# genome/breakdancer

Measured on AMD Instinct MI355X. Metric: read-pairs/s, records resident in HBM -> scored SV table (SURVEY 8d timing i); end to end from BAM: config.timings.bam_to_table (vs_baseline is taken there), higher is better.
Workload: dtype int32

## Files before the change

### breakdancer_amd/_lib.py

```python
import ctypes as C
import os

import numpy as np

_HERE = os.path.dirname(os.path.abspath(__file__))
LIB_PATH = os.path.join(_HERE, "libbdx.so")

OPT_FIELDS = ["min_len", "cut_sd", "max_sd", "min_map_qual", "min_read_pair", "seq_coverage_lim", "buffer_size",
              "transchr_rearrange", "fisher", "illumina_long_insert", "cn_lib", "print_af", "score_threshold",
              "chr_restricted"]


class bdx_opts(C.Structure):
    _fields_ = [(k, C.c_int32) for k in OPT_FIELDS]


class bdx_lib(C.Structure):
    _fields_ = [("mean_insertsize", C.c_float), ("std_insertsize", C.c_float), ("uppercutoff", C.c_float),
                ("lowercutoff", C.c_float), ("readlens", C.c_float), ("min_mapping_quality", C.c_int32),
                ("bam_index", C.c_int32)]


class bdx_batch(C.Structure):
    _fields_ = [(k, C.c_void_p) for k in ("tid", "pos", "mtid", "mpos", "isize", "flag", "qlen", "mapq", "lib", "bam",
# ... 11 lines not shown
                ("n_groups", C.c_uint32), ("n_svs", C.c_uint32), ("n_svs_printed", C.c_uint32)]


REGION_DTYPE = np.dtype([("tid", "<i4"), ("start", "<i4"), ("end", "<i4"), ("normal_read_pairs", "<i4"),
                         ("fwd_read_count", "<i4"), ("rev_read_count", "<i4"), ("n_reads", "<i4"), ("stored", "<i4"),
                         ("max_qlen", "<i4")])
SV_DTYPE = np.dtype([("chr", "<i4", 2), ("pos", "<i4", 2), ("fwd", "<i4", 2), ("rev", "<i4", 2), ("flag", "<i4"),
                     ("size", "<i4"), ("score", "<i4"), ("num_reads", "<i4"), ("printed", "<i4"), ("region", "<i4", 2),
                     ("lib_begin", "<i4"), ("lib_count", "<i4"), ("cn_begin", "<i4"), ("cn_count", "<i4"),
                     ("allele_frequency", "<f4"), ("logp", "<f8")])

EXPORTS = ["bdx_opts_default", "bdx_create", "bdx_destroy", "bdx_strerror", "bdx_last_error", "bdx_reserve", "bdx_push",
           "bdx_set_device_reads", "bdx_run", "bdx_get_summary", "bdx_get_counters", "bdx_get_regions", "bdx_get_svs",
           "bdx_get_sv_lists", "bdx_get_read_class", "bdx_get_timings", "bdx_classify", "bdx_poisson_log_upper_tail",
           "bdx_device", "bdx_stream", "bdx_set_collect_support", "bdx_get_sv_support",
           "bdx_set_host_walk", "bdx_set_debug", "bdx_use_name_check", "bdx_run_many", "bdx_get_walk_split", "bdx_trim_results", "bdx_set_stage_timing", "bdx_get_cross_window_svs",
           "bdx_set_enqueue_ahead", "bdx_was_replayed", "bdx_acquire_batch", "bdx_submit_batch", "bdx_reset_reads", "bdx_set_pass1_statistics",
           "bdx_warm_up", "bdx_set_process_option", "bdx_dist_unique_id", "bdx_dist_create", "bdx_dist_create_threads", "bdx_dist_destroy", "bdx_dist_last_error", "bdx_dist_rank",
           "bdx_dist_world", "bdx_dist_chromosome", "bdx_dist_run", "bdx_dist_result", "bdx_dist_set_collect_support", "bdx_dist_get_phase_ms", "bdx_dist_phase_name", "bdx_dist_prepare", "bdx_dist_reset_reads", "bdx_dist_get_exchange", "bdx_dist_get_collectives", "bdx_dist_set_debug", "bdx_dist_owner", "bdx_dist_plan",
           "bdx_bamdec_create", "bdx_bamdec_destroy", "bdx_bamdec_last_error", "bdx_bamdec_acquire", "bdx_bamdec_submit", "bdx_bamdec_progress",
           "bdx_bamdec_finish", "bdx_bamdec_rearm", "bdx_bamdec_fetch", "bdx_bamdec_stats", "bdx_bamdec_host_ms", "bdx_merge_decoded", "bdx_append_decoded", "bdx_inflate_blocks", "bdx_insert_size_stats",
           "bdx_count_junction_pairs", "bdx_bamdec_set_exclude", "bdx_bamdec_excluded", "bdx_exclude_mask", "bdx_count_site_pairs", "bdx_site_breakpoint_bounds", "bdx_count_interval_reads",
           "bdx_set_mark_duplicates", "bdx_get_duplicates", "bdx_dist_set_mark_duplicates", "bdx_dist_get_duplicates", "bdx_mark_duplicates"]

DUP_T = 64

SITE_DTYPE = np.dtype([("tid1", "<i4"), ("pos1", "<i4"), ("tid2", "<i4"), ("pos2", "<i4"), ("flag_mask", "<u4")])
SITE_BOUNDS_DTYPE = np.dtype([("n", "<u4"), ("lo1", "<i4"), ("hi1", "<i4"), ("lo2", "<i4"), ("hi2", "<i4")])
INTERVAL_DTYPE = np.dtype([("tid", "<i4"), ("beg", "<i4"), ("end", "<i4")])
DEPTH_CHUNK = 2048
SITE_FLAGS = (1 << 1) | (1 << 2) | (1 << 3) | (1 << 4) | (1 << 5) | (1 << 8)
# ... 32 lines not shown
    L.bdx_get_read_class.argtypes = [vp, vp, C.c_size_t]
    L.bdx_get_timings.argtypes = [vp, vp, C.c_int]
    L.bdx_set_host_walk.argtypes = [vp, C.c_int]
    L.bdx_set_debug.argtypes = [vp, C.c_char_p, C.c_int]
    L.bdx_use_name_check.argtypes = [vp, C.c_int]
    L.bdx_run_many.argtypes = [C.POINTER(vp), C.c_size_t, C.c_int]
    L.bdx_set_stage_timing.argtypes = [vp, C.c_int]
    L.bdx_set_enqueue_ahead.argtypes = [vp, C.c_int]
    L.bdx_was_replayed.argtypes = [vp]
    L.bdx_acquire_batch.argtypes = [vp, C.c_size_t, C.POINTER(bdx_batch_buf)]
    L.bdx_submit_batch.argtypes = [vp, C.c_size_t]
    L.bdx_reset_reads.argtypes = [vp]
    L.bdx_set_pass1_statistics.argtypes = [vp, vp, C.c_uint32]
    L.bdx_get_walk_split.argtypes = [vp, vp, vp, vp]
    L.bdx_get_cross_window_svs.argtypes = [vp, vp]
    L.bdx_classify.argtypes = [C.POINTER(bdx_opts), C.POINTER(bdx_lib), C.c_int, C.POINTER(bdx_batch), vp, C.c_int]
    L.bdx_poisson_log_upper_tail.argtypes = [vp, vp, vp, C.c_size_t, C.c_int]
    L.bdx_device.argtypes = [vp]
    L.bdx_stream.argtypes = [vp]
    L.bdx_stream.restype = vp
    L.bdx_set_collect_support.argtypes = [vp, C.c_int]
    L.bdx_get_sv_support.argtypes = [vp, vp, vp, vp, C.c_size_t, vp]
    L.bdx_count_junction_pairs.argtypes = [vp, vp, vp, vp, C.c_size_t, C.c_int, vp]
    L.bdx_count_site_pairs.argtypes = [vp, vp, C.c_size_t, C.c_int32, C.c_int, vp]
    L.bdx_site_breakpoint_bounds.argtypes = [vp, vp, C.c_size_t, C.c_int32, vp]
    L.bdx_count_interval_reads.argtypes = [vp, vp, C.c_size_t, C.c_int, vp]
    L.bdx_set_mark_duplicates.argtypes = [vp, C.c_int]
    L.bdx_get_duplicates.argtypes = [vp, vp, vp]
    L.bdx_dist_set_mark_duplicates.argtypes = [vp, C.c_int]
    L.bdx_dist_get_duplicates.argtypes = [vp, vp, vp]
# ... 4 lines not shown
```

### breakdancer_amd/api.py

```python
import ctypes as C
from dataclasses import dataclass

import numpy as np

from . import _lib as L

FLAG_NAMES = ["NA", "ARP_FF", "ARP_LARGE_INSERT", "ARP_SMALL_INSERT", "ARP_RF", "ARP_RR", "NORMAL_FR", "NORMAL_RF",
              "ARP_CTX", "MATE_UNMAPPED", "UNMAPPED"]


class BdxError(RuntimeError):
    pass


@dataclass
class Options:
    min_len: int = 7
    cut_sd: int = 3
    max_sd: int = 1000000000
    min_map_qual: int = 35
    min_read_pair: int = 2
    seq_coverage_lim: int = 1000
    buffer_size: int = 100
    transchr_rearrange: bool = False
# ... 301 lines not shown
        return self

    def walk_split(self):
        v = [C.c_uint32(0), C.c_uint32(0), C.c_uint32(0)]
        self._chk(self.lib.bdx_get_walk_split(self.h, C.byref(v[0]), C.byref(v[1]), C.byref(v[2])), "bdx_get_walk_split")
        return tuple(x.value for x in v)

    def was_replayed(self):
        return bool(self.lib.bdx_was_replayed(self.h))

    def cross_window_svs(self):
        v = C.c_uint32(0)
        self._chk(self.lib.bdx_get_cross_window_svs(self.h, C.byref(v)), "bdx_get_cross_window_svs")
        return v.value

    def timings(self):
        ms = np.zeros(12, np.float32)
        self.lib.bdx_get_timings(self.h, ms.ctypes.data_as(C.c_void_p), 12)
        return dict(zip(("classify", "compact", "regions", "join", "readback", "walk", "score", "total", "final_wait", "merge",
                         "combine_scores"), ms.tolist()))


def mark_duplicates(tid, pos, mtid, mpos, flag, lib, name_key, device=0):
    lb = L.load()
    cols = [np.ascontiguousarray(a, dtype=dt) for a, dt in ((tid, np.int32), (pos, np.int32), (mtid, np.int32), (mpos, np.int32),
                                                            (flag, np.uint16), (lib, np.uint8), (name_key, np.uint64))]
    n = len(cols[0])
    if any(len(c) != n for c in cols):
        raise ValueError("the columns differ in length")
    out = np.zeros(n, np.uint8)
# ... 18 lines not shown
```

### breakdancer_amd/csrc/bdx_api.hip

```cpp
#include <hip/hip_runtime.h>

#include <algorithm>
#include <atomic>
#include <functional>
#include <memory>
#include <chrono>
#include <cmath>
#include <cstdio>
#include <cstddef>
#include <cstring>
#include <string>
#include <thread>
#include <unordered_map>
#include <utility>
#include <vector>

#include "../../include/bdx.h"
#include "bdx_buf.h"
#include "bdx_dev.h"
#include "bdx_k3.h"
#include "bdx_shard.h"
#include "bdx_scan.h"
#include "bdx_walk.h"
#include "bdx_bam_dev.h"
// ... 38 lines not shown
    size_t n = 0, cap = 0;
    bool adopted = false;
    DevBuf b_tid, b_pos, b_mtid, b_mpos, b_isize, b_flag, b_qlen, b_mapq, b_lib, b_bam, b_key, b_check;
    bool groups_in_hbm = false;
    bool use_check = false;

    DevBuf b_libs, b_cls, b_tile_tot, b_tile_pre, b_tile_mono, b_blk_cnt, b_cnt, b_p1, b_fold, b_stash, b_chunk_tot, b_counts;
    DevBuf b_lib_mean, b_kdens;
    PinBuf h_p1, h_cnt, h_counts, h_terms;
    PinBuf h_hs_rec, h_hs_aux, h_hs_lists, h_printed;
    StageBufs sb;
    PinBuf h_flags;
    PinBuf h_count;
    uint32_t seq = 0;
    int dbg_no_stash = 0, dbg_max_chunks = 0, dbg_ins_plain = 0, dbg_gather_walk = 0, dbg_regions_copy = 0, dbg_asm_plain = 0, dbg_depth_plain = 0;
    uint32_t lb_seq = 0;
    float k1_ms_last = 0;
    bool k1_timed = false;
    bool stage_timing = false;
    bool poll = true;
    bool materialized = true;
    bool rows_packed = false;
    uint32_t n_sv_total = 0, n_groups_total = 0, n_terms_total = 0, n_cn_total = 0;
    Event ev_groups, ev_regions;
    int big_walk_mode = -1;
    int64_t last_big_groups = -1;
    FinalizeParams fp_deferred{};
    bool finalize2_deferred = false;
    bool bucketed_join = false;
    bool host_walk_only = false;
// ... 178 lines not shown

StageDims stage_dims(const bdx_ctx* c, uint32_t na) {
    StageDims d;
    d.na = na; d.nkeys = c->nkeys; d.nlibs = c->nlibs; d.use_check = c->use_check;
    d.k2_clears_join = c->force_direct_join || (!c->bucketed_join && na <= kDirectJoinMax);
    d.groups_in_hbm = c->groups_in_hbm; d.table_in_hbm = c->table_in_hbm; d.k6_cap = c->k6_cap;
    d.big_walk = c->big_walk_mode >= 0 ? c->big_walk_mode : (c->last_big_groups >= 0 ? (c->last_big_groups > 2000 ? 1 : 0) : -1);
    d.join_n = d.join_own = na; d.join_slots = d.k2_clears_join ? direct_join_slots(na) : 0;
    return d;
}

int pass1_prepare(bdx_ctx* c, uint32_t tiles_cap);
int presize_stages(bdx_ctx* c, const StageDims& dm);
int presize_stages_here(bdx_ctx* c, const StageDims& dm);
int pass1_classify(bdx_ctx* c, uint32_t upto, bool timed);

constexpr uint32_t kStreamTilesMin = 4096;

int enqueue_batch(bdx_ctx* c, const bdx_batch& b, bool lazy_keys) {
    if (c->n + b.n > c->cap) {
        BDX_TRY(alloc_reads(c, std::max(c->n + b.n, c->cap * 2)));
    }
    const size_t o = c->n, n = b.n;
    if (c->mark_dup && c->dup_done && o)
        return fail(c, BDX_ESTATE, "duplicates of this load are marked already: reads cannot be appended behind a run (bdx_reset_reads starts the next load)");
    hipStream_t s = c->copy_stream;
    if (o == 0) {
        c->key_segs.clear();
        const uint64_t tiles = (c->cap + kTile - 1) / kTile;
        if (tiles <= 0xFFFFFFFFull) {
// ... 391 lines not shown
    c->k1_done = 0;
    HIPCHK(c, c->b_cls.ensure(std::max<size_t>((size_t)tiles_cap * kTile, 16)));
    c->use_stash = !c->dbg_no_stash && nkeys <= kStashKeys;
    if (c->use_stash) HIPCHK(c, c->b_stash.ensure(std::max<size_t>((size_t)tiles_cap * kStashCap * sizeof(StashRec), 64)));
    HIPCHK(c, c->b_tile_tot.ensure((size_t)ncols * tstride * 4));
    HIPCHK(c, c->b_tile_pre.ensure((size_t)ncols * tstride * 4));
    HIPCHK(c, c->b_tile_mono.ensure((size_t)nbams * tstride * sizeof(MonoRec)));
    HIPCHK(c, c->b_blk_cnt.ensure((size_t)kCntCopies * ncnt * 4));
    HIPCHK(c, c->b_cnt.ensure((size_t)ncnt * 4));
    HIPCHK(c, c->b_p1.ensure(sizeof(Pass1)));
    HIPCHK(c, c->h_p1.ensure(sizeof(Pass1)));
    HIPCHK(c, c->h_cnt.ensure((size_t)ncnt * 4));
    HIPCHK(c, c->h_counts.ensure(sizeof(StageCounts)));
    HIPCHK(c, c->b_counts.ensure(sizeof(StageCounts)));
    HIPCHK(c, c->h_count.ensure((size_t)kMaxChunks * 8));
    const size_t w_tot = (size_t)ncols * tstride, w_mono = (size_t)nbams * tstride * sizeof(MonoRec) / 4;
    if (w_tot > 0xFFFFFFFFull || w_mono > 0xFFFFFFFFull) {
        HIPCHK(c, hipMemsetAsync(c->b_tile_tot.p, 0, w_tot * 4, s));
        HIPCHK(c, hipMemsetAsync(c->b_tile_mono.p, 0xFF, w_mono * 4, s));
    }
    InitList il{};
    int k = 0;
    auto add = [&](void* p, size_t words, uint32_t value) { il.ptr[k] = (uint32_t*)p; il.words[k] = (uint32_t)words; il.value[k] = value; ++k; };
    if (w_tot <= 0xFFFFFFFFull && w_mono <= 0xFFFFFFFFull) { add(c->b_tile_tot.p, w_tot, 0u); add(c->b_tile_mono.p, w_mono, 0xFFFFFFFFu); }
    add(c->b_blk_cnt.p, (size_t)kCntCopies * ncnt, 0u);
    add(c->b_p1.p, sizeof(Pass1) / 4, 0u);
    add(c->b_counts.p, sizeof(StageCounts) / 4, 0u);
    il.n = k;
    launch_init(il, s);
    return BDX_OK;
// ... 2 lines not shown
int pass1_classify(bdx_ctx* c, uint32_t upto, bool timed) {
    hipStream_t s = c->stream;
    if (upto <= c->k1_done) return BDX_OK;
    K1Params k1{};
    k1.r = c->d; k1.n = c->n; k1.ntiles = upto; k1.tstride = c->tstride; k1.tile0 = c->k1_done;
    k1.nlibs = c->nlibs; k1.nbams = c->nbams; k1.nkeys = c->nkeys;
    k1.max_sd = c->opts.max_sd; k1.opt_t = c->opts.transchr_rearrange; k1.opt_l = c->opts.illumina_long_insert;
    k1.libs = c->b_libs.as<DevLib>(); k1.cls = c->b_cls.as<uint8_t>(); k1.tile_tot = c->b_tile_tot.as<uint32_t>();
    k1.tile_mono = c->b_tile_mono.as<MonoRec>();
    k1.blk_cnt = c->b_blk_cnt.as<uint32_t>();
    k1.stash = c->use_stash ? c->b_stash.as<StashRec>() : nullptr;
    const uint32_t span = upto - c->k1_done;
    const int grid1 = (int)std::min<uint32_t>((span + kWaves - 1) / kWaves, (uint32_t)kK1MaxGrid);
    launch_k1(k1, grid1, k1_lds_bytes(c->nlibs, c->nbams, c->nkeys), s, timed ? c->ev[0] : nullptr, timed ? c->ev[1] : nullptr);
    c->k1_done = upto;
    return BDX_OK;
}

int do_pass1(bdx_ctx* c, uint32_t na_cap, bool wait, bool defer_second, bool post_count) {
    HIPCHK(c, hipSetDevice(c->device));
    hipStream_t s = c->stream;
    const int nlibs = c->nlibs, nbams = c->nbams, nkeys = c->nkeys;
    const int ncols = 2 + nkeys, ncnt = nlibs * kNumFlags + nlibs + nbams;
    if (c->n >= ((size_t)1 << 32)) return fail(c, BDX_ELIMIT, "more than 2^32 - 1 reads in one context (read indices and the prefix counters are 32-bit)");
    const uint32_t ntiles = (uint32_t)((c->n + kTile - 1) / kTile);
    c->ntiles = ntiles;
    c->ran = false; c->replayed = false;
    c->cls_n = (size_t)-1;
    c->na_alloc = 0;
    c->regions.clear(); c->r_pk.clear(); c->parts.clear();
    c->reg = nullptr; c->nreg = 0; c->rpk = nullptr;
    c->walk.clear();
    if (!c->walk_scratch) c->walk_scratch.reset(walk_scratch_new());
    c->n_printed = 0;
    memset(&c->counts, 0, sizeof(c->counts));
    for (float& m : c->stage_ms) m = 0;

    if (c->copy_pending) {
        HIPCHK(c, hipStreamWaitEvent(s, c->ev_copy, 0));
        c->copy_pending = false;
    }
    if (!(c->k1_live && c->k1_cap_tiles >= ntiles)) {
        BDX_TRY(pass1_prepare(c, ntiles));
    }
    c->k1_live = false;
    if (c->mark_dup && c->k1_done == 0) {
        BDX_TRY(mark_duplicates(c));
    }
    const uint32_t tstride = c->tstride;
    const bool time_k1 = (c->stage_timing || c->seq % kK1EventPeriod == 0) && c->k1_done == 0 && ntiles > 0;
    {
        BDX_TRY(pass1_classify(c, ntiles, time_k1));
    }
    FinalizeParams fp{};
    fp.ntiles = ntiles; fp.tstride = tstride; fp.nblk = 0;
    fp.nfold = std::max<uint32_t>(1, std::min<uint32_t>(64, (ntiles + 1023) / 1024));
    HIPCHK(c, c->b_fold.ensure((size_t)nbams * fp.nfold * sizeof(MonoRec)));
    fp.fold_part = c->b_fold.as<MonoRec>();
    fp.nlibs = nlibs; fp.nbams = nbams; fp.nkeys = nkeys; fp.ncols = ncols; fp.ncnt = ncnt; fp.w0 = c->w0;
    fp.tile_tot = c->b_tile_tot.as<uint32_t>(); fp.tile_pre = c->b_tile_pre.as<uint32_t>(); fp.tile_mono = c->b_tile_mono.as<MonoRec>();
    {
        const uint32_t nsuper = (ntiles + kK2TilesPerWave - 1) / kK2TilesPerWave;
        const uint32_t round = 4096;
        const uint32_t rounds = std::max<uint32_t>(1, (nsuper + round - 1) / round);
        const uint32_t max_chunks = c->dbg_max_chunks > 0 ? (uint32_t)std::min(c->dbg_max_chunks, (int)kMaxChunks) : (uint32_t)kMaxChunks;
        fp.chunk_super = round * ((rounds + max_chunks - 1) / max_chunks);
        fp.nchunk = std::max<uint32_t>(1, (nsuper + fp.chunk_super - 1) / fp.chunk_super);
        HIPCHK(c, c->b_chunk_tot.ensure((size_t)ncols * kMaxChunks * 8));
        fp.chunk_tot = c->b_chunk_tot.as<uint32_t>();
        fp.chunk_base = fp.chunk_tot + (size_t)ncols * kMaxChunks;
    }
    fp.blk_cnt = c->b_blk_cnt.as<uint32_t>(); fp.cnt = c->b_cnt.as<uint32_t>(); fp.p1 = c->b_p1.as<Pass1>();
    HIPCHK(c, c->b_kdens.ensure(64 * 4));
    fp.libs = c->b_libs.as<DevLib>(); fp.cn_lib = c->opts.cn_lib; fp.key_density = c->b_kdens.as<float>();
    fp.cnt_host = c->h_cnt.as<uint32_t>(); fp.p1_host = c->h_p1.as<Pass1>();
    memset(c->h_p1.p, 0, sizeof(Pass1));
    HIPCHK(c, c->h_flags.ensure(64));
    ++c->seq;
    fp.flag_host = c->h_flags.as<uint32_t>(); fp.flag_value = c->seq;
    fp.na_cap = na_cap;
    fp.count_host = post_count && c->poll ? c->h_count.as<uint64_t>() : nullptr; fp.count_stamp = c->seq;
    c->count_chunks = fp.count_host ? fp.nchunk : 0;
    c->fp_deferred = fp;
    c->finalize2_deferred = defer_second;
    launch_finalize(fp, s, !defer_second);
    c->k1_timed = time_k1;
    return wait ? wait_pass1(c) : BDX_OK;
}

int wait_pass1(bdx_ctx* c) {
    const int ncnt = c->nlibs * kNumFlags + c->nlibs + c->nbams;
    if (!wait_flag(c, 0, c->seq)) {
        HIPCHK(c, hipStreamSynchronize(c->stream));
        if (c->h_flags.p && *((volatile uint32_t*)c->h_flags.p) != c->seq) return fail(c, BDX_EINTERNAL, "the pass-1 record did not arrive: its kernel was not launched");
    }
    c->p1 = *c->h_p1.as<Pass1>();
    c->cnt_local.assign(c->h_cnt.as<uint32_t>(), c->h_cnt.as<uint32_t>() + ncnt);
    if (c->k1_timed) {
        float ms = 0;
        if (hipEventElapsedTime(&ms, c->ev[0], c->ev[1]) == hipSuccess) c->k1_ms_last = ms;
// ... 191 lines not shown
            k2.fill_ptr[3] = b.b_pair_lo.as<uint32_t>(); k2.fill_words[3] = na; k2.fill_value[3] = 0xFFFFFFFFu;
            c->join_table_clean = slots;
        }
        {
            size_t ns = 0;
            BDX_TRY(upload_key_segs(c, &ns));
            if (ns) {
                k2.nseg = (int)ns;
                k2.seg_begin = c->b_seg.as<uint64_t>();
                k2.seg_ptr = (const uint64_t* const*)(c->b_seg.as<uint64_t>() + ns + 1);
                k2.seg_qlen = (const uint16_t* const*)(c->b_seg.as<uint64_t>() + 2 * ns + 1);
                k2.seg_check = (const uint64_t* const*)(c->b_seg.as<uint64_t>() + 3 * ns + 1);
            }
        }
        launch_k2(k2, k2_lds_bytes(nkeys), s, c->finalize2_deferred ? &c->fp_deferred : nullptr);
        c->finalize2_deferred = false;
    }
    if (c->finalize2_deferred) {
        launch_finalize2_only(c->fp_deferred, s);
        c->finalize2_deferred = false;
    }
    if (c->stage_timing) HIPCHK(c, hipEventRecord(c->ev[3], s));
    return BDX_OK;
}

void own_borrowed_regions(bdx_ctx* c) {
    if (!c->reg || (const void*)c->reg != c->sb.h_regs.p) return;
    const HostRegion* r = c->reg;
    const uint32_t* pk = c->rpk;
    const size_t n = c->nreg;
    std::vector<HostRegion> keep(r, r + n);
    std::vector<uint32_t> keep_pk;
    if (pk) keep_pk.assign(pk, pk + n * 2 * (size_t)c->nkeys);
    c->regions.swap(keep); c->r_pk.swap(keep_pk);
// ... 100 lines not shown
    if (nr) memcpy(c->regions.data() + ph, rr, (size_t)nr * sizeof(RegionRec));
    c->r_pk.assign((size_t)ph * 2 * nkeys, 0u);
    c->r_pk.insert(c->r_pk.end(), pk, pk + (size_t)nr * 2 * nkeys);
    c->reg = c->regions.data(); c->nreg = c->regions.size(); c->rpk = c->r_pk.data();
}

void decode_groups(bdx_ctx* c, const GroupRec* gr, uint32_t ng, uint32_t ph) {
    c->parts.resize(ng);
    for (uint32_t i = 0; i < ng; ++i) {
        const uint64_t k = gr[i].key;
        c->parts[i] = GroupPart{(uint32_t)(k >> 38) + ph, (uint32_t)((k >> 12) & ((1u << 26) - 1)) + ph, (uint8_t)(k & 15),
                                (uint8_t)((k >> 4) & 255), gr[i].pairs, gr[i].sum_isize};
    }
}

int k6_prepare(bdx_ctx* c, bool force_host, int rounds) {
    hipStream_t s = c->stream;
    K6Arrays& a = c->k6;
    a = K6Arrays{};
    const StageDims dm = stage_dims(c, c->na_alloc);
    const uint32_t na = dm.k6_regions();
    if (!na) return BDX_OK;
    BDX_TRY(size_k6(c->sb, dm, s, &c->err));
    const StageBufs& b = c->sb;
    const K6Caps k = k6_caps(dm);
    const int nkeys = c->nkeys, nlibs = c->nlibs;
    const size_t cap = na, p2 = k.p2, svc = k.sv, nsort = k.nsort;
    a.sv_cap = k.sv; a.term_cap = k.term; a.cn_cap = k.cn; a.lib_stride = k.lib_stride;
    a.old_key = b.b_ins.as<uint64_t>(); a.hs_key_dev = a.old_key + p2;
    a.old_slot = (uint32_t*)(a.hs_key_dev + svc); a.ins_T = a.old_slot + p2; a.ins_src = a.ins_T + svc + 1;
    a.ins_pre_l = a.ins_src + svc + 1; a.ins_pre_c = a.ins_pre_l + svc + 1;
    a.sorted_key = (uint64_t*)(((uintptr_t)(a.ins_pre_c + svc + 1) + 7) & ~(uintptr_t)7); a.sorted_slot = (uint32_t*)(a.sorted_key + nsort);
    a.rank_part = a.sv_cap > 2048u ? a.sorted_slot + nsort : nullptr;
    a.sv_begin = b.b_sv_src.as<uint2>(); a.sv_src = (uint32_t*)(a.sv_begin + a.sv_cap); a.ltail = b.b_ltail.as<double>();
    a.d_lib_index = b.b_dlists.as<int32_t>(); a.d_cn_key = a.d_lib_index + a.term_cap; a.d_cn_value = (float*)(a.d_cn_key + a.cn_cap);
    a.cap = na;
    a.r_rec = c->k6_r_rec ? c->k6_r_rec : b.b_r_rec.as<RegionRec>(); a.r_pk = c->k6_r_pk ? c->k6_r_pk : b.b_r_pk.as<uint32_t>();
    a.taint = c->k6_taint;
    a.region_of = c->k3.region_of; a.partner = c->k4.partner; a.pair_lo = c->k4.pair_lo; a.meta = c->cp.meta; a.isize = c->cp.isize;
    a.in_groups = c->k6_in_groups; a.in_goff = c->k6_in_goff; a.first_of = c->k6_in_groups ? c->k6_in_goff : nullptr;
    a.parts = b.b_parts.as<PartRec>();
    a.rs = b.b_rs.as<RegSum>();
    a.out_deg = b.b_out_deg.as<uint32_t>(); a.label = a.out_deg + cap; a.bad_v = a.out_deg + 2 * cap; a.bad = a.out_deg + 3 * cap;
    a.mcount = a.out_deg + 4 * cap; a.pcount = a.out_deg + 5 * cap;
    a.members = b.b_members.as<MemberInfo>();
    a.own_nsv = b.b_own.as<uint32_t>(); a.own_nacc = a.own_nsv + cap; a.own_ncn = a.own_nsv + 2 * cap; a.own_first = a.own_nsv + 3 * cap; a.slot_next = a.own_nsv + 4 * cap; a.owners = a.own_nsv + 5 * cap; a.owners_big = a.own_nsv + 6 * cap; a.emit_part = a.own_nsv + 7 * cap;
    a.big_walk = dm.walks_big();
    a.member_ids = a.big_walk ? b.b_member_ids.as<uint32_t>() : nullptr;
// ... 32 lines not shown
        if (c->k3.host_copy_later) a.flag_regions = c->h_flags.as<uint32_t>() + 3;
        a.mirror_in_walk = force_host ? 0 : 1;
    }
    return BDX_OK;
}

void k6_pairs(bdx_ctx* c) {
    if (c->k6.cap) launch_k6_pairs(c->k6, c->k6.cap, c->stream);
}
int k6_then_walk(bdx_ctx* c, void (*first)(const K6Arrays&, uint32_t, hipStream_t)) {
    const K6Arrays& a = c->k6;
    if (!a.cap) return BDX_OK;
    first(a, a.cap, c->stream);
    if (!c->poll) BDX_TRY(signal_ready(c, 1, c->ev_groups));
    launch_k6_walk(a, a.cap, c->stream);
    return BDX_OK;
}

int presize_stages(bdx_ctx* c, const StageDims& dm) {
    struct Guard {
        bdx_ctx* c;
        explicit Guard(bdx_ctx* c_) : c(c_) { c->sizing.fetch_add(1, std::memory_order_acq_rel); c->sizing_err.clear(); }
        ~Guard() { c->sizing.fetch_sub(1, std::memory_order_acq_rel); }
    } guard(c);
    std::string* err = &c->sizing_err;
    SZCHK(hipSetDevice(c->device));
    own_borrowed_regions(c);
    BDX_TRY(size_compact(c->sb, dm, err));
    BDX_TRY(size_cut(c->sb, dm, c->stream, err));
    BDX_TRY(size_join(c->sb, dm, err));
// ... 106 lines not shown
    static_assert(sizeof(HostSv) == sizeof(SvOut) && offsetof(HostSv, grp_mask) == offsetof(SvOut, grp_mask) &&
                      offsetof(HostSv, start) == offsetof(SvOut, start), "SV record layout");
    c->n_sv_host = (uint32_t)c->walk.svs.size();
    c->n_groups_total = c->walk.n_groups + c->counts.n_groups_dev;
    const StageCounts c2 = *c->sb.h_counts2.as<StageCounts>();
    if (c2.overflow) return fail(c, BDX_EINTERNAL, "SV list overflow");
    c->n_sv_total = c2.n_sv_dev; c->n_terms_total = c2.n_terms_dev; c->n_cn_total = c2.n_cn_dev;
    c->counts.n_sv_dev = c2.n_sv_dev - c->n_sv_host;
    {
        const uint32_t g = c->k6.printed_host ? k6_score_grid(c->k6) : 0u;
        const uint32_t* pb = c->k6.printed_host;
        uint32_t np = 0;
        for (uint32_t i = 0; i < g; ++i) np += pb[i];
        c->n_printed = np;
    }
    c->counts.n_old = c2.n_old;
    c->materialized = false;
    if (c->opts.fisher && !c->table_in_hbm) {
        materialize(c);
        finish_scores(c->opts, c->log_tail.data(), c->walk.svs.data(), c->walk.svs.size(), &c->n_printed);
    }
    const auto tf2 = std::chrono::steady_clock::now();
    c->stage_ms[8] = ms_between(tf0, tf1);
    c->stage_ms[9] = ms_between(tf1, tf2);
    c->stage_ms[10] = 0;
    c->ran = true;
    return BDX_OK;
}

int host_walk(bdx_ctx* c, int32_t last_maxq, bool any_anomalous) {
    HIPCHK(c, hipSetDevice(c->device));
// ... 484 lines not shown
    if (out.ensure(n) != hipSuccess) return BDX_ENOMEM;
    KdParams p{};
    p.tid = col[0].as<int32_t>(); p.pos = col[1].as<int32_t>(); p.mtid = col[2].as<int32_t>(); p.mpos = col[3].as<int32_t>();
    p.flag = col[4].as<uint16_t>(); p.lib = col[5].as<uint8_t>(); p.key = col[6].as<uint64_t>(); p.n = n;
    uint64_t marked = 0, groups = 0;
    BDX_TRY(kd_run(nullptr, p, k, nullptr, out.as<uint8_t>(), nullptr, &marked, &groups));
    if (hipDeviceSynchronize() != hipSuccess || hipMemcpy(mask, out.p, n, hipMemcpyDeviceToHost) != hipSuccess) return BDX_EHIP;
    if (n_groups) *n_groups = groups;
    return BDX_OK;
}

int bdx_set_debug(bdx_ctx* c, const char* name, int value) {
    if (!c || !name) return BDX_EINVAL;
    struct { const char* n; int* p; } ints[] = {{"no_stash", &c->dbg_no_stash}, {"max_chunks", &c->dbg_max_chunks}, {"spec_test", &c->spec_test},
                                                 {"big_walk", &c->big_walk_mode}, {"ins_plain", &c->dbg_ins_plain}, {"regions_copy", &c->dbg_regions_copy},
                                                 {"asm_plain", &c->dbg_asm_plain}, {"gather_walk", &c->dbg_gather_walk}, {"depth_plain", &c->dbg_depth_plain}};
    for (auto& e : ints)
        if (!strcmp(name, e.n)) { *e.p = value; return BDX_OK; }
    if (!strcmp(name, "bucketed_join")) { c->bucketed_join = value != 0; return BDX_OK; }
    if (!strcmp(name, "no_poll")) { c->poll = value == 0; return BDX_OK; }
    return fail(c, BDX_EINVAL, std::string("unknown debug switch ") + name);
}

int bdx_set_host_walk(bdx_ctx* c, int on) {
    if (!c) return BDX_EINVAL;
    c->host_walk_only = on != 0;
    return BDX_OK;
}

int bdx_get_walk_split(const bdx_ctx* c, uint32_t* n_sv_device, uint32_t* n_sv_host, uint32_t* n_groups_host) {
    if (!c) return BDX_EINVAL;
    if (!c->ran) return BDX_ESTATE;
    if (n_sv_device) *n_sv_device = c->counts.n_sv_dev;
    if (n_sv_host) *n_sv_host = c->n_sv_host;
    if (n_groups_host) *n_groups_host = c->counts.n_groups;
    return BDX_OK;
}

int bdx_get_cross_window_svs(const bdx_ctx* c, uint32_t* n_sv_device) {
    if (!c || !n_sv_device) return BDX_EINVAL;
    if (!c->ran) return BDX_ESTATE;
    *n_sv_device = c->counts.n_old;
    return BDX_OK;
}

int bdx_set_pass1_statistics(bdx_ctx* c, const uint32_t* counters, uint32_t covered_ref_len) {
    if (!c) return BDX_EINVAL;
    if (!counters) { c->ov_cnt.clear(); return BDX_OK; }
    c->ov_cnt.assign(counters, counters + (size_t)c->nlibs * kNumFlags + c->nlibs + c->nbams);
    c->ov_covered = covered_ref_len;
    c->ran = false;
    return BDX_OK;
}

int bdx_was_replayed(const bdx_ctx* c) { return c && c->ran && c->replayed ? 1 : 0; }

int bdx_get_timings(const bdx_ctx* c, float* ms, int cap) {
// ... 182 lines not shown
```

### breakdancer_amd/csrc/bdx_dev.h

```cpp
#pragma once
#include <hip/hip_runtime.h>
#include <stdint.h>

namespace bdx {

constexpr int kTile = 256;
constexpr int kBlock = 256;
constexpr int kWaves = kBlock / 64;
constexpr int kNumFlags = 11;
constexpr int kK2TilesPerWave = 4;
constexpr int kCntCopies = 64;
constexpr int kMaxChunks = 64;
constexpr int kStashCap = 16;
constexpr int kStashKeys = 2;

struct StashRec {
    int32_t tid, pos, isize;
    uint32_t meta;
    uint32_t where;
    uint32_t proper;
    uint32_t pad[2];
};
static_assert(sizeof(StashRec) == 32, "two 16-byte stores");

// ... 44 lines not shown
    uint32_t key_tot[60];
    unsigned long long ref_len[256];
};

struct FinalizeParams {
    uint32_t ntiles, tstride, nblk;
    uint32_t nfold;
    MonoRec* fold_part;
    int nlibs, nbams, nkeys, ncols, ncnt;
    int w0;
    const uint32_t* tile_tot;
    uint32_t* tile_pre;
    uint32_t* chunk_tot;
    uint32_t* chunk_base;
    uint32_t chunk_super, nchunk;
    const MonoRec* tile_mono;
    const uint32_t* blk_cnt;
    uint32_t* cnt;
    Pass1* p1;
    uint32_t* cnt_host;
    Pass1* p1_host;
    const DevLib* libs;
    int cn_lib;
    float* key_density;
    uint32_t* flag_host;
    uint32_t flag_value;
    uint64_t* count_host;
    uint32_t count_stamp;
    uint32_t na_cap;
};

struct InitList {
// ... 171 lines not shown
```

### breakdancer_amd/csrc/bdx_finalize.h

```cpp
#pragma once
#include <cstddef>

#include "bdx_dev.h"

namespace bdx {

__device__ __forceinline__ MonoRec mono_combine(const MonoRec& a, const MonoRec& b) {
    if (a.ft == -1) return b;
    if (b.ft == -1) return a;
    MonoRec r;
    r.ft = a.ft; r.fp = a.fp; r.lt = b.lt; r.lp = b.lp;
    r.sum = a.sum + b.sum + (a.lt == b.ft ? (long long)b.fp - (long long)a.lp : 0ll);
    return r;
}
__device__ __forceinline__ MonoRec mono_shfl_down(const MonoRec& a, int o) {
    MonoRec r;
    r.ft = __shfl_down(a.ft, o); r.fp = __shfl_down(a.fp, o); r.lt = __shfl_down(a.lt, o); r.lp = __shfl_down(a.lp, o);
    r.sum = __shfl_down(a.sum, o);
    return r;
}

__device__ __forceinline__ void finalize2_body(const FinalizeParams& p) {
    __shared__ uint32_t s_acc[255 * 12 + 256];
    __shared__ unsigned long long s_ref[256];
    __shared__ uint32_t s_head[2];
    __shared__ uint32_t s_col[64];
    const int t = threadIdx.x, lane = t & 63, w = t >> 6;
    for (int i = t; i < p.ncnt; i += 256) s_acc[i] = 0;
    __syncthreads();
    for (int idx = t; idx < kCntCopies * p.ncnt; idx += 256) {
        const uint32_t v = p.blk_cnt[idx];
        if (v) atomicAdd(&s_acc[idx % p.ncnt], v);
    }
    __syncthreads();
    for (int i = t; i < p.ncnt; i += 256) {
        const uint32_t v = s_acc[i];
        p.cnt[i] = v;
        if (p.cnt_host) p.cnt_host[i] = v;
    }
    for (int c0 = 0; c0 < p.ncols; c0 += 4) {
        const int c = c0 + w;
        uint32_t v = (c < p.ncols && (uint32_t)lane < p.nchunk) ? p.chunk_tot[(size_t)c * kMaxChunks + lane] : 0u;
        {
            uint32_t inc = v;
#pragma unroll
            for (int o = 1; o < 64; o <<= 1) {
                const uint32_t u = __shfl_up(inc, o);
                if (lane >= o) inc += u;
// ... 87 lines not shown
```

### breakdancer_amd/csrc/bdx_insert.h

```cpp
#pragma once
#include "bdx_k3.h"
#include "bdx_scan.h"

namespace bdx {

constexpr int kKeyShiftT = 34, kKeyShiftStart = 7;
constexpr uint32_t kKeySeqMask = 127u;
static_assert(kK6MaxMembers * (kK6MaxMembers - 1) / 2 + (kK6MaxMembers - 1) <= (int)kKeySeqMask + 1, "k6_walk_kernel: the candidates of one component and window have sequence numbers of their own");

__device__ __forceinline__ uint32_t count_below(const uint32_t* v, uint32_t n, uint32_t x) {
    uint32_t lo = 0, hi = n;
    while (lo < hi) {
        const uint32_t mid = (lo + hi) / 2;
        if (v[mid] < x) lo = mid + 1; else hi = mid;
    }
    return lo;
}
__device__ __forceinline__ uint32_t count_below64(const uint64_t* v, uint32_t n, uint64_t x) {
    uint32_t lo = 0, hi = n;
    while (lo < hi) {
        const uint32_t mid = (lo + hi) / 2;
        if (v[mid] < x) lo = mid + 1; else hi = mid;
    }
    return lo;
}

constexpr uint32_t kInsLds = 2048;
constexpr uint32_t kInsThreads = 1024;
constexpr uint32_t kInsBucketMax = 8192;
constexpr uint32_t kInsCntLds = 10240;
constexpr uint32_t kInsBuckets = 2048;
constexpr uint32_t kInsBucketDepth = 128;
constexpr uint32_t kInsPerBucketPath = kInsBucketMax / kInsThreads;
constexpr uint32_t kInsSub = 64;
constexpr uint32_t kRankGrid = 256;
__device__ __forceinline__ void rank_layout(uint32_t nd, uint32_t* nchunk, uint32_t* nslice, uint32_t* per) {
    *nchunk = (nd + kScanBlock - 1) / kScanBlock;
    *nslice = min(kK6RankSlices, max(1u, kRankGrid / *nchunk));
    *per = (nd + *nslice - 1) / *nslice;
}

__device__ __forceinline__ uint64_t ins_bucket_span(uint32_t n_regions, uint32_t period) {
    const uint32_t nwin = n_regions / period + 2;
    return (uint64_t)nwin * kInsSub + 1;
// ... 291 lines not shown
```

### breakdancer_amd/csrc/bdx_k3.h

```cpp
#pragma once
#include "../../include/bdx.h"
#include "bdx_dev.h"

namespace bdx {

struct U4;

struct StageCounts {
    uint32_t n_cand;
    uint32_t n_regions;
    int32_t last_maxq;
    uint32_t n_pairs;
    uint32_t n_groups;
    uint32_t n_entries;
    uint32_t overflow;
    uint32_t n_printed;
    uint32_t n_sv_dev;
    uint32_t n_terms_dev;
    uint32_t n_cn_dev;
    uint32_t n_groups_dev;
    uint32_t stage_sv;
    uint32_t stage_lib;
    uint32_t stage_cn;
    uint32_t n_owners;
    uint32_t n_owners_big;
    uint32_t n_groups_big;
    uint32_t n_old;
    uint32_t n_ins;
    uint32_t sort_done;
    uint32_t irregular;
};

struct RegionRec {
    int32_t tid, start, end;
    uint32_t n, rev, nonctx, nnormal;
    int32_t maxq;
    uint32_t first;
};

struct GroupRec {
    uint64_t key;
    uint32_t pairs;
    uint32_t sum_isize;
};
// ... 95 lines not shown
    k ^= k >> 29;
    return (uint32_t)(k % world);
}
struct GatherPackage { uint64_t regions_off, pk_off, groups_off; uint32_t nr, ng; };
struct GatherDesc { GatherPackage p[kMaxRanks]; int world; };
void launch_k8_place_regions(const char* all, const GatherDesc& D, uint32_t max_nr, const uint64_t* rbase, int ntids, int nkeys2, RegionRec* r_rec,
                             uint32_t* r_pk, uint32_t* err, hipStream_t s);

void launch_k5(const double* lambda, const int32_t* k, double* out, uint32_t n, hipStream_t s);

constexpr int kK6MaxMembers = 4;
constexpr int kK6MaxIn = 3;
constexpr int kK6BigMembers = 64;
constexpr int kK6LibStride = 16;
constexpr int kK6LabelRoundsBig = 8;
constexpr uint32_t kK6RankSlices = 16;
constexpr uint32_t kK6RankSortMax = 1u << 17;
constexpr int kK6LabelRounds = 2;
constexpr int kK6LabelRoundsGather = 3;

struct RegSum {
    uint32_t np_all;
    uint32_t np_emit;
    uint32_t np_self;
    uint32_t w_self;
    uint32_t n_in;
    uint32_t n_pairs;
    uint32_t n_weak;
    uint32_t big;
    uint32_t e_lo[kK6MaxIn];
// ... 149 lines not shown
```

### breakdancer_amd/csrc/k1_classify.hip

```cpp
#include <cstddef>

#include <hip/hip_ext.h>

#include "bdx_dev.h"
#include "bdx_finalize.h"

#include <limits.h>

#ifdef BDX_KPROF
#include "bdx_scan.h"
#else
#define KPROF(row, col) do {} while (0)
#endif

namespace bdx {

constexpr int kMixedLibs = 8;

typedef int v4i __attribute__((ext_vector_type(4)));
typedef unsigned short v4us __attribute__((ext_vector_type(4)));
typedef unsigned char v4uc __attribute__((ext_vector_type(4)));
__device__ __forceinline__ int4 ldnt(const int32_t* p) { const v4i v = __builtin_nontemporal_load((const v4i*)p); return make_int4(v.x, v.y, v.z, v.w); }
__device__ __forceinline__ ushort4 ldnt(const uint16_t* p) { const v4us v = __builtin_nontemporal_load((const v4us*)p); return make_ushort4(v.x, v.y, v.z, v.w); }
__device__ __forceinline__ uchar4 ldnt(const uint8_t* p) { const v4uc v = __builtin_nontemporal_load((const v4uc*)p); return make_uchar4(v.x, v.y, v.z, v.w); }
// ... 631 lines not shown
            }
            __syncthreads();
            if (t == 0) s_carry += s_round;
            __syncthreads();
        }
        if (t == 0) p.chunk_tot[(size_t)c * kMaxChunks + g] = s_carry;
        KPROF(blockIdx.x * 16 + w, 2);
        return;
    }

    const uint32_t fb = blockIdx.x - nscan;
    const uint32_t chunk = (p.ntiles + p.nfold - 1) / p.nfold;
    const uint32_t c0 = fb * chunk, c1 = min(c0 + chunk, p.ntiles);
    const uint32_t per = (chunk + kFinBlock - 1) / kFinBlock;
    for (int b = 0; b < p.nbams; ++b) {
        const MonoRec* mo = p.tile_mono + (size_t)b * p.tstride;
        MonoRec acc;
        acc.ft = -1; acc.fp = 0; acc.lt = 0; acc.lp = 0; acc.sum = 0;
        const uint32_t t0 = min(c0 + (uint32_t)t * per, c1), t1 = min(t0 + per, c1);
        for (uint32_t i = t0; i < t1; i += 8) {
            MonoRec e[8];
#pragma unroll
            for (int q = 0; q < 8; ++q) {
                if (i + q < t1) e[q] = mo[i + q];
                else e[q].ft = -1;
            }
#pragma unroll
            for (int q = 0; q < 8; ++q) acc = mono_combine(acc, e[q]);
        }
        if (acc.ft != -12345) KPROF(blockIdx.x * 16 + w, 1);
#pragma unroll
        for (int o = 1; o < 64; o <<= 1) {
            const MonoRec other = mono_shfl_down(acc, o);
            if (lane + o < 64 && ((lane & (2 * o - 1)) == 0)) acc = mono_combine(acc, other);
        }
        if (lane == 0) s_mono[w] = acc;
        __syncthreads();
        if (t == 0) {
            MonoRec tot = s_mono[0];
            for (int k = 1; k < kFinBlock / 64; ++k) tot = mono_combine(tot, s_mono[k]);
// ... 43 lines not shown
```

### include/bdx.h

```cpp
#ifndef BDX_H
#define BDX_H

#include <stddef.h>
#include <stdint.h>

#ifdef __cplusplus
extern "C" {
#endif

typedef struct bdx_ctx bdx_ctx;

enum {
    BDX_OK = 0,
    BDX_EINVAL = 1,
    BDX_ENOMEM = 2,
    BDX_EHIP = 3,
    BDX_ESTATE = 4,
    BDX_ELIMIT = 5,
    BDX_EINTERNAL = 6
};

enum {
    BDX_NA = 0, BDX_ARP_FF = 1, BDX_ARP_LARGE_INSERT = 2, BDX_ARP_SMALL_INSERT = 3, BDX_ARP_RF = 4, BDX_ARP_RR = 5,
    BDX_NORMAL_FR = 6, BDX_NORMAL_RF = 7, BDX_ARP_CTX = 8, BDX_MATE_UNMAPPED = 9, BDX_UNMAPPED = 10, BDX_NUM_FLAGS = 11
// ... 111 lines not shown
int bdx_set_collect_support(bdx_ctx* ctx, int on);
int bdx_get_sv_support(const bdx_ctx* ctx, uint32_t* sv_offsets, uint64_t* read_index, uint8_t* read_flag, size_t cap,
                       size_t* n_total);

int bdx_get_read_class(const bdx_ctx* ctx, uint8_t* out, size_t cap);

int bdx_get_timings(const bdx_ctx* ctx, float* ms, int cap);
int bdx_set_stage_timing(bdx_ctx* ctx, int on);
int bdx_set_enqueue_ahead(bdx_ctx* ctx, int on);

int bdx_set_host_walk(bdx_ctx* ctx, int on);
int bdx_set_debug(bdx_ctx* ctx, const char* name, int value);
int bdx_get_walk_split(const bdx_ctx* ctx, uint32_t* n_sv_device, uint32_t* n_sv_host, uint32_t* n_groups_host);
int bdx_trim_results(bdx_ctx* ctx);
int bdx_get_cross_window_svs(const bdx_ctx* ctx, uint32_t* n_sv_device);
int bdx_was_replayed(const bdx_ctx* ctx);

int bdx_warm_up(int device);
int bdx_set_process_option(const char* name, int value);

int bdx_classify(const bdx_opts* opts, const bdx_lib* libs, int nlibs, const bdx_batch* host_batch, uint8_t* cls_out,
                 int device);
int bdx_poisson_log_upper_tail(const double* lambda, const int32_t* k, double* out, size_t n, int device);

typedef struct bdx_dist bdx_dist;
typedef struct bdx_unique_id { char internal[128]; } bdx_unique_id;
int bdx_dist_unique_id(bdx_unique_id* out);
int bdx_dist_create(bdx_dist** out, const bdx_opts* opts, const bdx_lib* libs, int nlibs, int nbams, int ntids,
                    int max_read_window_size0, int device, int rank, int world, const bdx_unique_id* id);
int bdx_dist_create_threads(bdx_dist** out, const bdx_opts* opts, const bdx_lib* libs, int nlibs, int nbams, int ntids,
// ... 102 lines not shown
```

Measured before the change: 29.37 billion.

## Skip pass-1 table reinit via in-kernel self-clearing; gate rank-ahead sort launch

The finalize kernels now zero the block counters and the stage-count words, and reset mono records as they consume them. The host tracks whether the pass-1 tables are already clean and skips the memset/init launches on reuse, clearing only tail tiles with 2D memsets when the tile count shrinks. Separately, the k6 rank-ahead partition sort now runs only when a heuristic predicts it is needed (transchr mode, small buffer, large allocation, or many cross-window SVs from the previous run). Both changes cut kernel launches and memory traffic per run, at the cost of extra stores in finalize and added state-tracking complexity that could leave stale data if the tracking is wrong.

```diff
diff --git a/breakdancer_amd/_lib.py b/breakdancer_amd/_lib.py
--- a/breakdancer_amd/_lib.py
+++ b/breakdancer_amd/_lib.py
@@ -49,7 +49,7 @@
            "bdx_set_device_reads", "bdx_run", "bdx_get_summary", "bdx_get_counters", "bdx_get_regions", "bdx_get_svs",
            "bdx_get_sv_lists", "bdx_get_read_class", "bdx_get_timings", "bdx_classify", "bdx_poisson_log_upper_tail",
            "bdx_device", "bdx_stream", "bdx_set_collect_support", "bdx_get_sv_support",
-           "bdx_set_host_walk", "bdx_set_debug", "bdx_use_name_check", "bdx_run_many", "bdx_get_walk_split", "bdx_trim_results", "bdx_set_stage_timing", "bdx_get_cross_window_svs",
+           "bdx_set_host_walk", "bdx_set_debug", "bdx_use_name_check", "bdx_run_many", "bdx_get_walk_split", "bdx_trim_results", "bdx_set_stage_timing", "bdx_get_cross_window_svs", "bdx_get_launch_counts",
            "bdx_set_enqueue_ahead", "bdx_was_replayed", "bdx_acquire_batch", "bdx_submit_batch", "bdx_reset_reads", "bdx_set_pass1_statistics",
            "bdx_warm_up", "bdx_set_process_option", "bdx_dist_unique_id", "bdx_dist_create", "bdx_dist_create_threads", "bdx_dist_destroy", "bdx_dist_last_error", "bdx_dist_rank",
            "bdx_dist_world", "bdx_dist_chromosome", "bdx_dist_run", "bdx_dist_result", "bdx_dist_set_collect_support", "bdx_dist_get_phase_ms", "bdx_dist_phase_name", "bdx_dist_prepare", "bdx_dist_reset_reads", "bdx_dist_get_exchange", "bdx_dist_get_collectives", "bdx_dist_set_debug", "bdx_dist_owner", "bdx_dist_plan",
@@ -112,6 +112,7 @@
     L.bdx_set_pass1_statistics.argtypes = [vp, vp, C.c_uint32]
     L.bdx_get_walk_split.argtypes = [vp, vp, vp, vp]
     L.bdx_get_cross_window_svs.argtypes = [vp, vp]
+    L.bdx_get_launch_counts.argtypes = [vp, vp]
     L.bdx_classify.argtypes = [C.POINTER(bdx_opts), C.POINTER(bdx_lib), C.c_int, C.POINTER(bdx_batch), vp, C.c_int]
     L.bdx_poisson_log_upper_tail.argtypes = [vp, vp, vp, C.c_size_t, C.c_int]
     L.bdx_device.argtypes = [vp]
diff --git a/breakdancer_amd/api.py b/breakdancer_amd/api.py
--- a/breakdancer_amd/api.py
+++ b/breakdancer_amd/api.py
@@ -339,6 +339,11 @@
         self._chk(self.lib.bdx_get_cross_window_svs(self.h, C.byref(v)), "bdx_get_cross_window_svs")
         return v.value
 
+    def launch_counts(self):
+        v = (C.c_uint32 * 2)()
+        self._chk(self.lib.bdx_get_launch_counts(self.h, v), "bdx_get_launch_counts")
+        return (int(v[0]), int(v[1]))
+
     def timings(self):
         ms = np.zeros(12, np.float32)
         self.lib.bdx_get_timings(self.h, ms.ctypes.data_as(C.c_void_p), 12)
diff --git a/breakdancer_amd/csrc/bdx_api.hip b/breakdancer_amd/csrc/bdx_api.hip
--- a/breakdancer_amd/csrc/bdx_api.hip
+++ b/breakdancer_amd/csrc/bdx_api.hip
@@ -76,6 +76,16 @@
     PinBuf h_count;
     uint32_t seq = 0;
     int dbg_no_stash = 0, dbg_max_chunks = 0, dbg_ins_plain = 0, dbg_gather_walk = 0, dbg_regions_copy = 0, dbg_asm_plain = 0, dbg_depth_plain = 0;
+    int dbg_rank_ahead = 0;
+    uint32_t last_cross = 0;
+    uint32_t n_init_launches = 0, n_rank_launches = 0;
+    struct Pass1Tables {
+        bool clean = false;
+        const void *tot = nullptr, *mono = nullptr, *blk = nullptr, *p1 = nullptr, *counts = nullptr;
+        uint32_t tstride = 0;
+        int ncols = 0, nbams = 0, ncnt = 0;
+        uint32_t high_tile = 0;
+    } p1t;
     uint32_t lb_seq = 0;
     float k1_ms_last = 0;
     bool k1_timed = false;
@@ -284,6 +294,7 @@
 int presize_stages(bdx_ctx* c, const StageDims& dm);
 int presize_stages_here(bdx_ctx* c, const StageDims& dm);
 int pass1_classify(bdx_ctx* c, uint32_t upto, bool timed);
+void pass1_consumed(bdx_ctx* c);
 
 constexpr uint32_t kStreamTilesMin = 4096;
 
@@ -705,6 +716,17 @@
     HIPCHK(c, c->h_counts.ensure(sizeof(StageCounts)));
     HIPCHK(c, c->b_counts.ensure(sizeof(StageCounts)));
     HIPCHK(c, c->h_count.ensure((size_t)kMaxChunks * 8));
+    {
+        bdx_ctx::Pass1Tables& T = c->p1t;
+        const bool same = T.tot == c->b_tile_tot.p && T.mono == c->b_tile_mono.p && T.blk == c->b_blk_cnt.p && T.p1 == c->b_p1.p &&
+                          T.counts == c->b_counts.p && T.tstride == tstride && T.ncols == ncols && T.nbams == nbams && T.ncnt == ncnt;
+        if (T.clean && same && tiles_cap >= T.high_tile) return BDX_OK;
+        T.tot = c->b_tile_tot.p; T.mono = c->b_tile_mono.p; T.blk = c->b_blk_cnt.p; T.p1 = c->b_p1.p; T.counts = c->b_counts.p;
+        T.tstride = tstride; T.ncols = ncols; T.nbams = nbams; T.ncnt = ncnt;
+        T.high_tile = 0;
+        T.clean = true;
+        ++c->n_init_launches;
+    }
     const size_t w_tot = (size_t)ncols * tstride, w_mono = (size_t)nbams * tstride * sizeof(MonoRec) / 4;
     if (w_tot > 0xFFFFFFFFull || w_mono > 0xFFFFFFFFull) {
         HIPCHK(c, hipMemsetAsync(c->b_tile_tot.p, 0, w_tot * 4, s));
@@ -737,8 +759,22 @@
     const int grid1 = (int)std::min<uint32_t>((span + kWaves - 1) / kWaves, (uint32_t)kK1MaxGrid);
     launch_k1(k1, grid1, k1_lds_bytes(c->nlibs, c->nbams, c->nkeys), s, timed ? c->ev[0] : nullptr, timed ? c->ev[1] : nullptr);
     c->k1_done = upto;
-    return BDX_OK;
-}
+    c->p1t.clean = false;
+    c->p1t.high_tile = std::max(c->p1t.high_tile, upto);
+    return BDX_OK;
+}
+
+int pass1_clear_tails(bdx_ctx* c, uint32_t ntiles) {
+    bdx_ctx::Pass1Tables& T = c->p1t;
+    const size_t w = T.high_tile - ntiles;
+    HIPCHK(c, hipMemset2DAsync(c->b_tile_tot.as<uint32_t>() + ntiles, (size_t)T.tstride * 4, 0, w * 4, (size_t)T.ncols, c->stream));
+    HIPCHK(c, hipMemset2DAsync(c->b_tile_mono.as<MonoRec>() + ntiles, (size_t)T.tstride * sizeof(MonoRec), 0xFF, w * sizeof(MonoRec), (size_t)T.nbams, c->stream));
+    T.high_tile = ntiles;
+    ++c->n_init_launches;
+    return BDX_OK;
+}
+
+void pass1_consumed(bdx_ctx* c) { c->p1t.clean = true; }
 
 int do_pass1(bdx_ctx* c, uint32_t na_cap, bool wait, bool defer_second, bool post_count) {
     HIPCHK(c, hipSetDevice(c->device));
@@ -765,6 +801,8 @@
     }
     if (!(c->k1_live && c->k1_cap_tiles >= ntiles)) {
         BDX_TRY(pass1_prepare(c, ntiles));
+    } else if (ntiles < c->p1t.high_tile) {
+        BDX_TRY(pass1_clear_tails(c, ntiles));
     }
     c->k1_live = false;
     if (c->mark_dup && c->k1_done == 0) {
@@ -794,6 +832,7 @@
         fp.chunk_base = fp.chunk_tot + (size_t)ncols * kMaxChunks;
     }
     fp.blk_cnt = c->b_blk_cnt.as<uint32_t>(); fp.cnt = c->b_cnt.as<uint32_t>(); fp.p1 = c->b_p1.as<Pass1>();
+    fp.counts = c->b_counts.as<uint32_t>(); fp.counts_words = (uint32_t)(sizeof(StageCounts) / 4);
     HIPCHK(c, c->b_kdens.ensure(64 * 4));
     fp.libs = c->b_libs.as<DevLib>(); fp.cn_lib = c->opts.cn_lib; fp.key_density = c->b_kdens.as<float>();
     fp.cnt_host = c->h_cnt.as<uint32_t>(); fp.p1_host = c->h_p1.as<Pass1>();
@@ -807,6 +846,7 @@
     c->fp_deferred = fp;
     c->finalize2_deferred = defer_second;
     launch_finalize(fp, s, !defer_second);
+    if (!defer_second) pass1_consumed(c);
     c->k1_timed = time_k1;
     return wait ? wait_pass1(c) : BDX_OK;
 }
@@ -1028,10 +1068,12 @@
             }
         }
         launch_k2(k2, k2_lds_bytes(nkeys), s, c->finalize2_deferred ? &c->fp_deferred : nullptr);
+        if (c->finalize2_deferred) pass1_consumed(c);
         c->finalize2_deferred = false;
     }
     if (c->finalize2_deferred) {
         launch_finalize2_only(c->fp_deferred, s);
+        pass1_consumed(c);
         c->finalize2_deferred = false;
     }
     if (c->stage_timing) HIPCHK(c, hipEventRecord(c->ev[3], s));
@@ -1162,6 +1204,12 @@
     }
 }
 
+bool ranks_ahead(const bdx_ctx* c) {
+    if (c->dbg_rank_ahead) return c->dbg_rank_ahead > 0;
+    return c->opts.transchr_rearrange || c->opts.buffer_size <= 3 || c->na_alloc >= (1u << 19) || c->last_cross > kK6RankAheadMin ||
+           c->k6_in_groups != nullptr || c->dbg_ins_plain == 1;
+}
+
 int k6_prepare(bdx_ctx* c, bool force_host, int rounds) {
     hipStream_t s = c->stream;
     K6Arrays& a = c->k6;
@@ -1179,7 +1227,7 @@
     a.old_slot = (uint32_t*)(a.hs_key_dev + svc); a.ins_T = a.old_slot + p2; a.ins_src = a.ins_T + svc + 1;
     a.ins_pre_l = a.ins_src + svc + 1; a.ins_pre_c = a.ins_pre_l + svc + 1;
     a.sorted_key = (uint64_t*)(((uintptr_t)(a.ins_pre_c + svc + 1) + 7) & ~(uintptr_t)7); a.sorted_slot = (uint32_t*)(a.sorted_key + nsort);
-    a.rank_part = a.sv_cap > 2048u ? a.sorted_slot + nsort : nullptr;
+    a.rank_part = a.sv_cap > 2048u && ranks_ahead(c) ? a.sorted_slot + nsort : nullptr;
     a.sv_begin = b.b_sv_src.as<uint2>(); a.sv_src = (uint32_t*)(a.sv_begin + a.sv_cap); a.ltail = b.b_ltail.as<double>();
     a.d_lib_index = b.b_dlists.as<int32_t>(); a.d_cn_key = a.d_lib_index + a.term_cap; a.d_cn_value = (float*)(a.d_cn_key + a.cn_cap);
     a.cap = na;
@@ -1242,6 +1290,7 @@
     first(a, a.cap, c->stream);
     if (!c->poll) BDX_TRY(signal_ready(c, 1, c->ev_groups));
     launch_k6_walk(a, a.cap, c->stream);
+    if (a.rank_part && !a.force_host) ++c->n_rank_launches;
     return BDX_OK;
 }
 
@@ -1378,7 +1427,7 @@
         for (uint32_t i = 0; i < g; ++i) np += pb[i];
         c->n_printed = np;
     }
-    c->counts.n_old = c2.n_old;
+    c->counts.n_old = c->last_cross = c2.n_old;
     c->materialized = false;
     if (c->opts.fisher && !c->table_in_hbm) {
         materialize(c);
@@ -1893,7 +1942,8 @@
     if (!c || !name) return BDX_EINVAL;
     struct { const char* n; int* p; } ints[] = {{"no_stash", &c->dbg_no_stash}, {"max_chunks", &c->dbg_max_chunks}, {"spec_test", &c->spec_test},
                                                  {"big_walk", &c->big_walk_mode}, {"ins_plain", &c->dbg_ins_plain}, {"regions_copy", &c->dbg_regions_copy},
-                                                 {"asm_plain", &c->dbg_asm_plain}, {"gather_walk", &c->dbg_gather_walk}, {"depth_plain", &c->dbg_depth_plain}};
+                                                 {"asm_plain", &c->dbg_asm_plain}, {"gather_walk", &c->dbg_gather_walk}, {"depth_plain", &c->dbg_depth_plain},
+                                                 {"rank_ahead", &c->dbg_rank_ahead}};
     for (auto& e : ints)
         if (!strcmp(name, e.n)) { *e.p = value; return BDX_OK; }
     if (!strcmp(name, "bucketed_join")) { c->bucketed_join = value != 0; return BDX_OK; }
@@ -1920,6 +1970,12 @@
     if (!c || !n_sv_device) return BDX_EINVAL;
     if (!c->ran) return BDX_ESTATE;
     *n_sv_device = c->counts.n_old;
+    return BDX_OK;
+}
+
+int bdx_get_launch_counts(const bdx_ctx* c, uint32_t out[2]) {
+    if (!c || !out) return BDX_EINVAL;
+    out[0] = c->n_init_launches; out[1] = c->n_rank_launches;
     return BDX_OK;
 }
 
diff --git a/breakdancer_amd/csrc/bdx_dev.h b/breakdancer_amd/csrc/bdx_dev.h
--- a/breakdancer_amd/csrc/bdx_dev.h
+++ b/breakdancer_amd/csrc/bdx_dev.h
@@ -82,8 +82,10 @@
     uint32_t* chunk_tot;
     uint32_t* chunk_base;
     uint32_t chunk_super, nchunk;
-    const MonoRec* tile_mono;
-    const uint32_t* blk_cnt;
+    MonoRec* tile_mono;
+    uint32_t* blk_cnt;
+    uint32_t* counts;
+    uint32_t counts_words;
     uint32_t* cnt;
     Pass1* p1;
     uint32_t* cnt_host;
diff --git a/breakdancer_amd/csrc/bdx_finalize.h b/breakdancer_amd/csrc/bdx_finalize.h
--- a/breakdancer_amd/csrc/bdx_finalize.h
+++ b/breakdancer_amd/csrc/bdx_finalize.h
@@ -30,8 +30,9 @@
     __syncthreads();
     for (int idx = t; idx < kCntCopies * p.ncnt; idx += 256) {
         const uint32_t v = p.blk_cnt[idx];
-        if (v) atomicAdd(&s_acc[idx % p.ncnt], v);
+        if (v) { atomicAdd(&s_acc[idx % p.ncnt], v); p.blk_cnt[idx] = 0u; }
     }
+    if (p.counts && (uint32_t)t < p.counts_words) p.counts[t] = 0u;
     __syncthreads();
     for (int i = t; i < p.ncnt; i += 256) {
         const uint32_t v = s_acc[i];
diff --git a/breakdancer_amd/csrc/bdx_insert.h b/breakdancer_amd/csrc/bdx_insert.h
--- a/breakdancer_amd/csrc/bdx_insert.h
+++ b/breakdancer_amd/csrc/bdx_insert.h
@@ -28,6 +28,7 @@
 constexpr uint32_t kInsLds = 2048;
 constexpr uint32_t kInsThreads = 1024;
 constexpr uint32_t kInsBucketMax = 8192;
+static_assert(kInsBucketMax == kK6RankAheadMin, "the rule that launches the rank sort (ranks_ahead, bdx_api.hip) goes by this length");
 constexpr uint32_t kInsCntLds = 10240;
 constexpr uint32_t kInsBuckets = 2048;
 constexpr uint32_t kInsBucketDepth = 128;
diff --git a/breakdancer_amd/csrc/bdx_k3.h b/breakdancer_amd/csrc/bdx_k3.h
--- a/breakdancer_amd/csrc/bdx_k3.h
+++ b/breakdancer_amd/csrc/bdx_k3.h
@@ -27,7 +27,6 @@
     uint32_t n_groups_big;
     uint32_t n_old;
     uint32_t n_ins;
-    uint32_t sort_done;
     uint32_t irregular;
 };
 
@@ -153,6 +152,7 @@
 constexpr int kK6BigMembers = 64;
 constexpr int kK6LibStride = 16;
 constexpr int kK6LabelRoundsBig = 8;
+constexpr uint32_t kK6RankAheadMin = 8192;
 constexpr uint32_t kK6RankSlices = 16;
 constexpr uint32_t kK6RankSortMax = 1u << 17;
 constexpr int kK6LabelRounds = 2;
diff --git a/breakdancer_amd/csrc/k1_classify.hip b/breakdancer_amd/csrc/k1_classify.hip
--- a/breakdancer_amd/csrc/k1_classify.hip
+++ b/breakdancer_amd/csrc/k1_classify.hip
@@ -669,7 +669,7 @@
     const uint32_t c0 = fb * chunk, c1 = min(c0 + chunk, p.ntiles);
     const uint32_t per = (chunk + kFinBlock - 1) / kFinBlock;
     for (int b = 0; b < p.nbams; ++b) {
-        const MonoRec* mo = p.tile_mono + (size_t)b * p.tstride;
+        MonoRec* mo = p.tile_mono + (size_t)b * p.tstride;
         MonoRec acc;
         acc.ft = -1; acc.fp = 0; acc.lt = 0; acc.lp = 0; acc.sum = 0;
         const uint32_t t0 = min(c0 + (uint32_t)t * per, c1), t1 = min(t0 + per, c1);
@@ -679,6 +679,11 @@
             for (int q = 0; q < 8; ++q) {
                 if (i + q < t1) e[q] = mo[i + q];
                 else e[q].ft = -1;
+            }
+            if (p.nbams > 1) {
+#pragma unroll
+                for (int q = 0; q < 8; ++q)
+                    if (i + q < t1 && e[q].ft != -1) mo[i + q].ft = -1;
             }
 #pragma unroll
             for (int q = 0; q < 8; ++q) acc = mono_combine(acc, e[q]);
diff --git a/include/bdx.h b/include/bdx.h
--- a/include/bdx.h
+++ b/include/bdx.h
@@ -149,6 +149,7 @@
 int bdx_get_walk_split(const bdx_ctx* ctx, uint32_t* n_sv_device, uint32_t* n_sv_host, uint32_t* n_groups_host);
 int bdx_trim_results(bdx_ctx* ctx);
 int bdx_get_cross_window_svs(const bdx_ctx* ctx, uint32_t* n_sv_device);
+int bdx_get_launch_counts(const bdx_ctx* ctx, uint32_t out[2]);
 int bdx_was_replayed(const bdx_ctx* ctx);
 
 int bdx_warm_up(int device);
```

Result: faster. 29.74 billion (median of 4 runs) (+1.3%).
